# dguilliams3/book-recommendation-engine

Hardware: AMD Instinct MI355X
Metric: exact top-10 queries/sec at 10M×1536 fp32 (1/8 GPU) + % HBM/MFMA roofline (higher is better)
Workload: dtype fp32

## Files before the change

### book-recommendation-engine_amd/csrc/vs_api.hip

```cpp
#include <algorithm>
#include <cstdio>
#include <cstring>
#include <mutex>
#include <shared_mutex>
#include <string>
#include <vector>

#include "../../include/vsearch.h"
#include "vs_internal.h"

using namespace vs;

constexpr int kI8FirstBackoff = 8;
constexpr int kI8MaxBackoff = 64;

struct vs_index {
  int d = 0;
  int metric = VS_METRIC_L2;
  int dtype = VS_DTYPE_F32;
  int device = 0;
  int esize = 4;
  int64_t ld = 0;
  int64_t ntotal = 0;
  int64_t capacity = 0;
// ... 693 lines not shown
                           : (int)std::max<int64_t>(1, std::min<int64_t>(ntiles, (512 + nqt - 1) / nqt));
  part.P = 2 * nsplit;
  const size_t n = (size_t)a.nq_pad * part.P * KP;
  VS_HIP(scr.alloc((void**)&part.key, n * sizeof(float)), "vs: scratch");
  VS_HIP(scr.alloc((void**)&part.id, n * sizeof(int)), "vs: scratch");
  const void* qmat = a.qb16 ? a.qb16 : (const void*)a.qbuf;
  {
    KernelTimer tm(st, qlist ? nullptr : "gemm_topk");
    VS_HIP(launch_gemm_topk(KP, a.mode, idx->codes, a.xaux, qmat, a.qaux, idx->ld, idx->esize,
                            ntotal, a.nq_pad, nsplit, a.self0, part, st, qlist, qcount),
           "vs: gemm_topk launch");
    tm.stop();
  }
  VS_HIP(launch_merge_partials(a.mode, part, qlist ? a.nq_pad : a.nq, a.k, idx->id_base,
                               a.min_score, a.D, a.I, a.k, st, a.raw, qlist, qcount),
         "vs: merge launch");
  return VS_OK;
}

int adaptive_record(vs_index* idx, const int* handed, int n, hipStream_t st);
int run_paged(vs_index* idx, const SearchArgs& a, hipStream_t st, const int* gl = nullptr,
              const int* gc = nullptr);
int run_gemm_rescored(vs_index* idx, const SearchArgs& a, int need, int KF, int plane,
                      hipStream_t st, const int* gl, const int* gc);

static bool dump_enabled() {
  static const bool v = [] {
    const char* e = getenv("VS_X1_DUMP");
    return !e || atoi(e) != 0;
  }();
  return v;
}

static int recut_mode() {
  const char* e = getenv("VS_X1_RECUT");
  const int v = e ? atoi(e) : 1;
  return v == 0 ? 0 : v == 2 ? 2 : 1;
}

constexpr int64_t kSmallFilterMinRows = 1 << 18;
bool small_filter_on() {
  const char* e = getenv("VS_SMALL_FILTER");
  return !e || atoi(e) != 0;
}
bool small_l2d_ok(int mode, const SearchArgs& a) {
  if (!(mode == MODE_L2 && a.l2_direct)) return true;
  const char* e = getenv("VS_SMALL_L2D");
  return !e || atoi(e) != 0;
}

bool skinny_deep_on() {
  const char* e = getenv("VS_SKINNY_DEEP");
  return !e || atoi(e) != 0;
}

static int x1_wg_target(int nqt) {
  const char* e = getenv("VS_X1_WGS");
  const int v = e ? atoi(e) : 0;
  return v > 0 ? v : nqt <= 8 ? 256 : 512;
}

static bool tail_wait_on(const SearchArgs& a, hipStream_t st) {
  const char* e = getenv("VS_TAIL_WAIT");
  if (e && atoi(e) == 0) return false;
  if (a.host_wait) return true;
  hipStreamCaptureStatus cs = hipStreamCaptureStatusNone;
// ... 139 lines not shown
  }
  x.xaux = a.xaux;
  x.QH = QH;
  x.qs = qs;
  x.qaux = qaux;
  x.nqa = qa_rows;
  x.ld = !aug ? idx->ld : i8 ? idx->ld + idx->aug_m : idx->ld + kAugBf16;
  x.ntotal = ntotal;
  x.self0 = self_rows ? a.self0 : -1;
  x.qrow = qrow;
  x.qcount = gc;
  const BoundArgs ba = aug ? make_bound_args_l2aug(idx->ld, idx->aug, plane)
                           : make_bound_args(idx->ld, plane);
  if (!gathered && !small && x1_dump_applies(kmode, plane) && dump_enabled() &&
      x1_pass_dumps(ntotal, x.nsplit)) {
    const int64_t lists = (int64_t)x.nq_pad * part.P;
    const int dR = (int)std::min<int64_t>(x1_dump_slots(), (int64_t(4) << 30) / (lists * 8));
    if (dR >= 16) {
      int *dc = nullptr, *ds = nullptr;
      hipError_t e = scr.alloc((void**)&dc, (size_t)lists * sizeof(int));
      if (e == hipSuccess) e = scr.alloc((void**)&ds, (size_t)lists * dR * 2 * sizeof(int));
      if (e == hipSuccess) {
        VS_HIP(scr.alloc((void**)&x.qcut, (size_t)qa_rows * sizeof(float)), "vs: scratch");
        double* bk = nullptr;
        VS_HIP(scr.alloc((void**)&bk, (size_t)qa_rows * sizeof(double)), "vs: scratch");
        VS_HIP(hipMemsetD32Async((hipDeviceptr_t)x.qcut, 0x7f7fffff, (size_t)qa_rows, st),
               "vs: cuts");
        VS_HIP(hipMemsetAsync(dc, 0, (size_t)lists * sizeof(int), st), "vs: dumps");
        VS_HIP(launch_qbound(mode, Q, idx->ld, qaux, plane, stats, qr2, qa_rows, bk, st, &ba),
               "vs: cuts");
        x.qbkey = bk;
        x.qcut_m = need;
        x.dump = true;
        x.recut = recut_mode();
        x.dcount = dc;
        x.dslot = ds;
        x.dR = dR;
        x.dstats = device_stats(idx->device) ? device_stats(idx->device) + 6 : nullptr;
      } else {
        (void)hipGetLastError();
      }
    }
  }
  {
    KernelTimer whole(st, gathered ? nullptr : i8 ? "gemm_topk_x1_i8_pass" : "gemm_topk_x1_pass",
                      false);
    X1SpanTimer tm(i8 ? "gemm_topk_x1_i8" : "gemm_topk_x1",
                   i8 ? "gemm_topk_x1_i8_list" : "gemm_topk_x1_list");
    if (!gathered) x.timing = &tm;
    if (gathered && deep && !i8 && kmode == MODE_IP && a.self0 < 0 && skinny_deep_on()) {
      VS_HIP(launch_skinny_plane(FILTER_BF16, x.XH, x.QH, x.ld, ntotal, gc, nullptr, nullptr, part,
                                 st),
             "vs: skinny deep stage");
      x.qskip = skinny_plane_max_queries();
    }
    if (small) {
      int* cnt = nullptr;
      VS_HIP(scr.alloc((void**)&cnt, sizeof(int)), "vs: scratch");
      VS_HIP(hipMemsetD32Async((hipDeviceptr_t)cnt, a.nq, 1, st), "vs: count");
      KernelTimer ks(st, i8 ? "skinny_plane_topk_i8" : "skinny_plane_topk");
      VS_HIP(launch_skinny_plane(plane, x.XH, x.QH, x.ld, ntotal, cnt, qs, x.xs, part, st, a.nq),
             "vs: skinny first stage");
      ks.stop();
    } else {
      int nd = 0;
      VS_HIP(launch_gemm_topk_x1(kmode, x, part, st, &nd), "vs: gemm_topk_x1 launch");
// ... 1357 lines not shown
```

### book-recommendation-engine_amd/csrc/vs_gemm_x1.hip

```cpp
#include <algorithm>
#include <climits>
#include <cmath>
#include <cstdlib>
#include <type_traits>

#include "vs_device.h"

#ifndef VS_X1_PROBE
#define VS_X1_PROBE 0
#endif
#define VS_X1_P(bit) ((VS_X1_PROBE & (bit)) != 0)

namespace vs {

#ifndef VS_X1_STAMP
#define VS_X1_STAMP 0
#endif
constexpr int kStampSeg = 9;
constexpr int kStampCnt = 3;
constexpr int kStampN = 2 * (kStampSeg + kStampCnt) + 2;
__device__ unsigned long long g_x1_stamps[kStampN];

namespace {

constexpr int kT = 256;
constexpr int kNbuf = 5;
constexpr int kX1ChunkTiles = 64;
constexpr int kDumpMaxR = 128;
#ifndef VS_X1_SCHED_I8
#define VS_X1_SCHED_I8 0
#endif
#ifndef VS_X1_SEGDMA
#define VS_X1_SEGDMA 0
#endif
constexpr int x1_sched(int el, bool dump, bool hyb = false) {
  return el != FILTER_I8 ? 2 : VS_X1_SCHED_I8 ? VS_X1_SCHED_I8 : dump || hyb ? 2 : 1;
}
constexpr bool x1_has_dump(int mode, int el) {
  return mode == MODE_IP || (mode == MODE_COS && el == FILTER_I8);
}
static bool x1_cos_dump_on() {
  const char* e = getenv("VS_X1_COSDUMP");
  return e && atoi(e) != 0;
}

__device__ __forceinline__ unsigned long long stamp_now() {
  unsigned long long t;
  __builtin_amdgcn_sched_barrier(0);
  asm volatile("s_memtime %0\n\ts_waitcnt lgkmcnt(0)" : "=s"(t)::"memory");
  __builtin_amdgcn_sched_barrier(0);
  return t;
}

__device__ __forceinline__ f32x4 row4(const float* __restrict__ p) { return *(const f32x4*)p; }
__device__ __forceinline__ f32x4 row4(const uint16_t* __restrict__ p) {
  const uint2 u = *(const uint2*)p;
  return f32x4{__uint_as_float(u.x << 16), __uint_as_float(u.x & 0xFFFF0000u),
               __uint_as_float(u.y << 16), __uint_as_float(u.y & 0xFFFF0000u)};
}

__device__ __forceinline__ bf16x8 as_bf(const uint4& u) { return __builtin_bit_cast(bf16x8, u); }
__device__ __forceinline__ i32x4 as_i4(const uint4& u) { return __builtin_bit_cast(i32x4, u); }

template <int EL>
using AccT = typename std::conditional<EL == FILTER_I8, i32x16, f32x16>::type;
template <int EL>
__device__ __forceinline__ AccT<EL> mfma_blk(const uint4& a, const uint4& b, const AccT<EL>& c) {
  if constexpr (EL == FILTER_I8)
    return __builtin_amdgcn_mfma_i32_32x32x32_i8(as_i4(a), as_i4(b), c, 0, 0, 0);
  else
    return __builtin_amdgcn_mfma_f32_32x32x16_bf16(as_bf(a), as_bf(b), c, 0, 0, 0);
}

// ... 19 lines not shown
}

__device__ __forceinline__ float sel4x4(const f32x4 (&v)[4], int i) {
  float r = v[0][0];
#pragma unroll
  for (int j = 1; j < 16; ++j) r = i == j ? v[j >> 2][j & 3] : r;
  return r;
}

__device__ __forceinline__ int i8_threshold(float lim, float c) {
  const float q = lim * __builtin_amdgcn_rcpf(c);
  const float qm = q > 0.0f ? q * (1.0f - 0x1p-20f) : q * (1.0f + 0x1p-20f);
  float fl = floorf(qm) - 2.0f;
  fl = fminf(fmaxf(fl, -2147483520.0f), 2147483520.0f);
  const int T = (int)fl;
  return (float)T * c <= lim ? T : INT_MIN;
}

__device__ __forceinline__ float sel16(const f32x16& v, int i) {
  float r = v[0];
#pragma unroll
  for (int j = 1; j < 16; ++j) r = i == j ? v[j] : r;
  return r;
}

template <int EL>
__device__ __forceinline__ float x1_key(int sum_bits, float qsc, float fx) {
  if constexpr (EL == FILTER_I8) return -((float)sum_bits * (qsc * fx));
  else return -__int_as_float(sum_bits);
}

}

template <int KR, int MODE, bool DUMP, int EL, bool HYB = false>
__global__ __launch_bounds__(512, 1) void gemm_topk_x1(
    const char* __restrict__ XH, const float* __restrict__ xs, const float* __restrict__ xaux,
    const char* __restrict__ QH, const float* __restrict__ qs, const float* __restrict__ qaux,
    int nqa, int nksteps, int ntotal, int ntiles, int nsplit, int nqt, int qtile0, int64_t self0,
    const int* __restrict__ qrow, const int* __restrict__ qcount, int chunk, int chunk_end,
    int nchunk, int KP, int qg, float* __restrict__ pkey, int* __restrict__ pid,
    const float* __restrict__ xgmax, const float* __restrict__ xgmin, const float* __restrict__ qcut,
    int* __restrict__ dcount, int* __restrict__ dslot, int dR, int qskip) {
  static_assert(!DUMP || x1_has_dump(MODE, EL), "dump form");
  static_assert(!HYB || (!DUMP && x1_has_dump(MODE, EL)), "hybrid launch");
  constexpr int NBUF = kNbuf;
  constexpr int kStepB = kT * 64;
  constexpr int D = NBUF - 1;
  static_assert(NBUF * 2 * kStepB <= 160 * 1024, "LDS");
  __shared__ __attribute__((aligned(16))) char smem[NBUF * 2 * kStepB];

  const int tid = threadIdx.x;
  const int lane = tid & 63;
  const int w = __builtin_amdgcn_readfirstlane(tid >> 6);
  const int h = lane >> 5;
  const int c32 = lane & 31;
  const int wr = w & 1;
  const int wq = w >> 1;

  int qt, sp;
  {
    const int nblk = gridDim.x;
    const int b = blockIdx.x;
    const int qga = qg < 0 ? -qg : qg;
    const int QG = nqt < qga ? nqt : qga;
    const int G = nqt / QG;
    const int S = nblk >> 3;
    if ((nblk & 7) == 0 && nqt * nsplit == nblk && nqt % QG == 0 && G <= 8 && 8 % G == 0 &&
        S % QG == 0) {
      const int xcd = b & 7, slot = b >> 3, DG = S / QG;
      qt = (xcd % G) * QG + slot % QG;
      sp = (xcd / G) * DG + slot / QG;
    } else if (qg > 0 && (nblk & 7) == 0 && nqt * nsplit == nblk && nqt % QG == 0 && G % 8 == 0) {
      const int xcd = b & 7, slot = b >> 3, per = QG * nsplit;
      const int gi = slot / per, rem = slot - gi * per;
      qt = (gi * 8 + xcd) * QG + rem % QG;
      sp = rem / QG;
    } else {
      const int xcd = b & 7, slot = b >> 3, qq = nblk >> 3, rr = nblk & 7;
      const int lb = (xcd < rr ? xcd * (qq + 1) : rr * (qq + 1) + (xcd - rr) * qq) + slot;
      qt = lb % nqt;
      sp = lb / nqt;
    }
  }
  if (qcount && (qt * kT >= *qcount || *qcount <= qskip)) return;
  const int s0 = (int)((int64_t)sp * ntiles / nsplit);
  const int s1 = (int)((int64_t)(sp + 1) * ntiles / nsplit);
  const int t0 = s0 + (int)((int64_t)(s1 - s0) * chunk / nchunk);
  const int t1 = s0 + (int)((int64_t)(s1 - s0) * chunk_end / nchunk);
  const int tsw = HYB ? t0 + (t1 - t0 + 3) / 4 : t1;

  int gq[2], selfrow[2];
  float qa[2], qsc[2];
#pragma unroll
  for (int qb = 0; qb < 2; ++qb) {
    gq[qb] = qt * kT + 64 * wq + 32 * qb + c32;
    qa[qb] = 0.0f;
    if constexpr (MODE == MODE_L2 || (MODE == MODE_COS && EL != FILTER_I8))
      qa[qb] = gq[qb] < nqa ? qaux[gq[qb]] : 0.0f;
    qsc[qb] = 0.0f;
    if constexpr (EL == FILTER_I8) qsc[qb] = gq[qb] < nqa ? qs[gq[qb]] : 0.0f;
    selfrow[qb] = qrow ? (gq[qb] < nqa ? qrow[gq[qb]] : -1) : self0 >= 0 ? (int)(self0 + gq[qb]) : -1;
  }
  const int P = nsplit * 4;
  const int pl = sp * 4 + wr * 2 + h;
  constexpr int KL = KR;
  float lk[2][KL];
  int li[2][KL];
  float tq[2] = {0.0f, 0.0f};
  int dc[2] = {0, 0};
#pragma unroll
  for (int qb = 0; qb < 2; ++qb) {
    if constexpr (DUMP) {
      const int64_t o = ((int64_t)gq[qb] * P + pl) * KP + KR - 1;
      float tl = qcut[gq[qb]];
      if (pid[o] >= 0) tl = fminf(tl, pkey[o]);
      tq[qb] = gq[qb] < nqa ? tl : -FLT_MAX;
      dc[qb] = dcount[(int64_t)gq[qb] * P + pl];
      asm volatile("" ::"v"(tq[qb]), "v"(dc[qb]));
    } else {
      const int64_t o = ((int64_t)gq[qb] * P + pl) * KP;
      if (chunk == 0) {
        list_init<KR, int>(lk[qb], li[qb]);
      } else {
#pragma unroll
        for (int e = 0; e < KR; ++e) {
          lk[qb][e] = pkey[o + e];
          li[qb][e] = pid[o + e];
        }
      }
#pragma unroll
      for (int e = 0; e < KR; ++e) asm volatile("" ::"v"(lk[qb][e]), "v"(li[qb][e]));
    }
    asm volatile("" ::"v"(qa[qb]));
    if constexpr (EL == FILTER_I8) asm volatile("" ::"v"(qsc[qb]));
  }

  if (t1 > t0) {
    const uint32_t soff = (uint32_t)(lane >> 2) * 64u + (uint32_t)((lane & 3) ^ (lane >> 4)) * 16u;
    const int fsw = (c32 >> 2) & 3;
    const char* qtile = QH + (int64_t)(qtile0 + qt) * nksteps * kStepB + (uint32_t)(32 * w) * 64u;
    const uint32_t lds0 = (uint32_t)(uintptr_t)VS_LDS(smem);
    const int nsteps = (t1 - t0) * nksteps;

    int ls = 0, lt = t0, lk_ = 0, lbuf = 0;
    uint32_t xlane = 0;
    int xhi = 0;
    auto set_xoff = [&](int tt) {
      const int f = tile_perm(tt);
      const int ln = (int)__builtin_amdgcn_mbcnt_hi(~0u, __builtin_amdgcn_mbcnt_lo(~0u, 0u));
      xhi = f & 0xF0;
      xlane = (uint32_t)((ln >> 2) ^ (f & 0x0C)) * 64u + (uint32_t)((ln & 3) ^ (ln >> 4)) * 16u;
    };
    set_xoff(t0);
    constexpr bool kSeg = x1_sched(EL, DUMP, HYB) == 2 && MODE == MODE_IP;
    const char* xstep = nullptr;
    const char* qstep = nullptr;
    uint32_t xl0 = 0, xl2 = 0;
    auto set_step_ptrs = [&]() {
      const int r0 = (32 * w) ^ xhi, r2 = (32 * w + 16) ^ xhi;
      xstep = XH + ((int64_t)lt * nksteps + lk_) * kStepB + (uint32_t)(r0 & ~16) * 64u;
      qstep = qtile + (int64_t)lk_ * kStepB;
      xl0 = xlane + (uint32_t)(r0 & 16) * 64u;
      xl2 = xlane + (uint32_t)(r2 & 16) * 64u;
    };
    if constexpr (kSeg) set_step_ptrs();

    int Tq[2] = {0, 0};
    float fm = 0.0f, fn = FLT_MAX;
    auto set_Tq = [&]() {
#pragma unroll
      for (int qb = 0; qb < 2; ++qb) {
        const float c = qsc[qb] * fm, cn = qsc[qb] * fn, last = tq[qb];
        Tq[qb] = (c > 0.0f && -last >= 0.0f)                    ? i8_threshold(-last, c)
                 : (cn > 0.0f && cn <= FLT_MAX && -last < 0.0f) ? min(i8_threshold(-last, cn), -1)
                 : (c > 0.0f || -0.0f < last)                   ? INT_MIN
                                                                : INT_MAX;
        asm volatile("" ::"v"(Tq[qb]));
      }
    };
    auto set_factor_bounds = [&](int ta) {
      const int ln = (int)__builtin_amdgcn_mbcnt_hi(~0u, __builtin_amdgcn_mbcnt_lo(~0u, 0u));
      for (int g = 16 * ta + ln; g < 16 * t1; g += 64) {
        fm = fmaxf(fm, xgmax[g]);
        fn = fminf(fn, xgmin[g]);
      }
#pragma unroll
      for (int m = 32; m >= 1; m >>= 1) {
        fm = fmaxf(fm, __shfl_xor(fm, m));
        fn = fminf(fn, __shfl_xor(fn, m));
      }
    };
    if constexpr (DUMP && EL == FILTER_I8) {
      set_factor_bounds(t0);
      set_Tq();
    }
    auto to_dump_mode = [&]() {
      if constexpr (HYB) {
        const int ln = (int)__builtin_amdgcn_mbcnt_hi(~0u, __builtin_amdgcn_mbcnt_lo(~0u, 0u));
        const int pl1 = sp * 4 + wr * 2 + (ln >> 5);
#pragma unroll
        for (int qb = 0; qb < 2; ++qb) {
          const int64_t g = (int64_t)(qt * kT + 64 * wq + 32 * qb + (ln & 31)) * P + pl1;
          const int64_t o = g * KP;
#pragma unroll
// ... 16 lines not shown
        }
      }
    };

    AccT<EL> acc[4][2];
    uint4 fa0[4], fb0[2], fa1[4], fb1[2];
    auto rd = [&](int buf, int s2, uint4 (&fa)[4], uint4 (&fb)[2]) {
      const char* base = smem + buf * 2 * kStepB;
      const int co = ((2 * s2 + h) ^ fsw) * 16;
      const char* cX = base + (128 * wr + c32) * 64 + co;
      const char* cQ = base + kStepB + (64 * wq + c32) * 64 + co;
      if constexpr (!VS_X1_P(2)) {
        fb[0] = *(const uint4*)cQ;
        fb[1] = *(const uint4*)(cQ + 32 * 64);
#pragma unroll
        for (int rb = 0; rb < 4; ++rb) fa[rb] = *(const uint4*)(cX + rb * 32 * 64);
      } else {
        auto opq = [](uint4& u) { asm volatile("" : "+v"(u.x), "+v"(u.y), "+v"(u.z), "+v"(u.w)); };
        asm volatile("" ::"v"(cX), "v"(cQ));
        opq(fb[0]);
        opq(fb[1]);
#pragma unroll
        for (int rb = 0; rb < 4; ++rb) opq(fa[rb]);
      }
    };
    auto mfma_rb = [&](int rb, const uint4 (&fa)[4], const uint4 (&fb)[2]) {
      acc[rb][0] = mfma_blk<EL>(fa[rb], fb[0], acc[rb][0]);
      acc[rb][1] = mfma_blk<EL>(fa[rb], fb[1], acc[rb][1]);
    };
    auto mfma_rb_first = [&](int rb, const uint4 (&fa)[4], const uint4 (&fb)[2]) {
      const AccT<EL> z = {};
      acc[rb][0] = mfma_blk<EL>(fa[rb], fb[0], z);
      acc[rb][1] = mfma_blk<EL>(fa[rb], fb[1], z);
    };
    auto stage_piece = [&](int i) {
      const char* xbase = XH + ((int64_t)lt * nksteps + lk_) * kStepB +
                          (uint32_t)((32 * w + 16 * (i >> 1)) ^ xhi) * 64u;
      const char* qbase = qtile + (int64_t)lk_ * kStepB + (uint32_t)(16 * (i >> 1)) * 64u;
      const uint32_t lx = lds0 + (uint32_t)lbuf * (2 * kStepB) + (uint32_t)(2 * w) * 1024u;
      if constexpr (!VS_X1_P(1)) {
        if ((i & 1) == 0) {
          if constexpr (!VS_X1_P(16))
            glds16(xbase, xlane, __builtin_amdgcn_readfirstlane(lx + (i >> 1) * 1024u));
        } else {
          if constexpr (!VS_X1_P(32))
            glds16(qbase, soff, __builtin_amdgcn_readfirstlane(lx + kStepB + (i >> 1) * 1024u));
        }
      } else {
        asm volatile("" ::"v"(xlane), "v"(soff), "s"(xbase), "s"(qbase), "s"(lx));
      }
    };
    auto advance_cursor = [&]() {
      if (ls + 1 < nsteps) {
        ++ls;
        if constexpr (kSeg) {
          xstep += kStepB;
          qstep += kStepB;
        }
        if (++lk_ == nksteps) {
          lk_ = 0;
          set_xoff(++lt);
          if constexpr (kSeg) set_step_ptrs();
        }
      }
      lbuf = lbuf + 1 == NBUF ? 0 : lbuf + 1;
    };
// ... 216 lines not shown
                list_insert<KR, int>(lk[qb], li[qb], sel16(key, bi), row);
              }
            } else {
              const float last = lim(qb);
              if constexpr (EL == FILTER_I8) {
                const float c = qsc[qb] * fmx[rb];
                const int T = (c > 0.0f && -last >= 0.0f) ? i8_threshold(-last, c) : INT_MIN;
#pragma unroll
                for (int r = 0; r < 16; ++r) cm |= (uint32_t)(acc[rb][qb][r] > T) << r;
              } else {
#pragma unroll
                for (int r = 0; r < 16; ++r) cm |= (uint32_t)(-acc[rb][qb][r] < last) << r;
              }
              while (cm) {
                const int bi = __builtin_ctz(cm);
                cm &= cm - 1;
                const int row = rowof(rb, bi >> 2) + (bi & 3);
                float key;
                if constexpr (EL == FILTER_I8)
                  key = x1_key<EL>(sel16i(acc[rb][qb], bi), qsc[qb], sel4x4(rv[r2], bi));
                else
                  key = -sel16(acc[rb][qb], bi);
                const bool ok = (plain || (row < ntotal && row != selfrow[qb])) && key < lim(qb);
                if (ok) list_insert<KR, int>(lk[qb], li[qb], key, row);
              }
            }
          }
        }
        VS_X1_EMARK(8);
      }
      }
    };

    constexpr int kSched = x1_sched(EL, DUMP, HYB);
    if constexpr (kSched == 1) {

#pragma unroll
    for (int i = 0; i < D; ++i) {
#pragma unroll
      for (int j = 0; j < 4; ++j) stage_piece(j);
      advance_cursor();
    }
    asm volatile("s_waitcnt vmcnt(12)" ::: "memory");
    __builtin_amdgcn_s_barrier();
    asm volatile("" ::: "memory");
    rd(0, 0, fa0, fb0);
    int buf = 0;
    const bool lag = w >= 4;
#if VS_X1_STAMP
    tA = stamp_now();
#define VS_X1_MARK1(i) (tB = stamp_now(), sg[i] += tB - tA, tA = tB)
#else
#define VS_X1_MARK1(i) ((void)0)
#endif
    auto s1_step = [&](auto first_tag) {
      constexpr bool first = decltype(first_tag)::value;
      const int nbuf = buf + 1 == NBUF ? 0 : buf + 1;
      if (lag) {
        asm volatile("s_waitcnt vmcnt(8)" ::: "memory");
        __builtin_amdgcn_s_barrier();
      }
      __builtin_amdgcn_sched_barrier(0);
      if constexpr (first) {
        mfma_rb_first(0, fa0, fb0);
        __builtin_amdgcn_sched_barrier(0);
        rd(buf, 1, fa1, fb1);
// ... 46 lines not shown
        }
        VS_X1_MARK1(5);
      }
    };
    if constexpr (HYB) {
      s1_tiles(t0, tsw, std::false_type{});
      to_dump_mode();
      s1_tiles(tsw, t1, std::true_type{});
    } else {
      s1_tiles(t0, t1, std::integral_constant<bool, DUMP>{});
    }
#undef VS_X1_MARK1
    } else {
    static_assert(NBUF == 5, "segmented schedule: 3 steps in flight over 5 images");
#pragma unroll
    for (int i = 0; i < 3; ++i) {
      stage_step();
      advance_cursor();
    }
    asm volatile("s_waitcnt vmcnt(8)" ::: "memory");
    __builtin_amdgcn_s_barrier();
    const bool lag = w >= 4;
    if (lag) __builtin_amdgcn_s_barrier();
    int buf = 0;
#if VS_X1_STAMP
    tA = stamp_now();
#define VS_X1_MARK(i) (tB = stamp_now(), sg[i] += tB - tA, tA = tB)
#else
#define VS_X1_MARK(i) ((void)0)
#endif
    auto seg_step = [&](auto first_tag) {
      constexpr bool first = decltype(first_tag)::value;
      __builtin_amdgcn_sched_barrier(0);
      rd(buf, 0, fa0, fb0);
      rd(buf, 1, fa1, fb1);
      __builtin_amdgcn_sched_barrier(0);
#if !VS_X1_SEGDMA
      stage_step();
      advance_cursor();
      __builtin_amdgcn_sched_barrier(0);
      VS_X1_MARK(0);
      asm volatile("s_waitcnt vmcnt(8)" ::: "memory");
#else
      VS_X1_MARK(0);
      asm volatile("s_waitcnt vmcnt(4)" ::: "memory");
#endif
      VS_X1_MARK(1);
      __builtin_amdgcn_s_barrier();
      __builtin_amdgcn_sched_barrier(0);
      VS_X1_MARK(2);
#if !VS_X1_SEGDMA
      if constexpr (first) {
#pragma unroll
        for (int rb = 0; rb < 4; ++rb) mfma_rb_first(rb, fa0, fb0);
      } else {
#pragma unroll
        for (int rb = 0; rb < 4; ++rb) mfma_rb(rb, fa0, fb0);
      }
#pragma unroll
      for (int rb = 0; rb < 4; ++rb) mfma_rb(rb, fa1, fb1);
#else
      {
        const uint32_t lx = __builtin_amdgcn_readfirstlane(lds0 + (uint32_t)lbuf * (2 * kStepB) +
                                                           (uint32_t)(2 * w) * 1024u);
        auto piece = [&](int j, uint32_t m0v, uint32_t voff, const char* sbase) {
          if constexpr (!kSeg) {
            stage_piece(j);
            return;
          }
          uint32_t keep;
          asm volatile(
              "s_mov_b32 %0, m0\n\ts_mov_b32 m0, %1\n\ts_nop 0\n\t"
              "global_load_lds_dwordx4 %2, %3\n\ts_mov_b32 m0, %0"
              : "=&s"(keep)
              : "s"(m0v), "v"(voff), "s"(sbase)
              : "memory");
        };
        static_assert(kStepB == 0x4000, "piece offsets");
        if constexpr (first) {
          mfma_rb_first(0, fa0, fb0);
          mfma_rb_first(1, fa0, fb0);
        } else {
          mfma_rb(0, fa0, fb0);
          mfma_rb(1, fa0, fb0);
        }
        __builtin_amdgcn_sched_barrier(0);
        piece(0, lx, xl0, xstep);
        __builtin_amdgcn_sched_barrier(0);
        if constexpr (first) {
          mfma_rb_first(2, fa0, fb0);
          mfma_rb_first(3, fa0, fb0);
        } else {
          mfma_rb(2, fa0, fb0);
          mfma_rb(3, fa0, fb0);
        }
        __builtin_amdgcn_sched_barrier(0);
        piece(1, lx + 0x4000u, soff, qstep);
        __builtin_amdgcn_sched_barrier(0);
        mfma_rb(0, fa1, fb1);
        mfma_rb(1, fa1, fb1);
        __builtin_amdgcn_sched_barrier(0);
        piece(2, lx + 0x400u, xl2, xstep);
        __builtin_amdgcn_sched_barrier(0);
        mfma_rb(2, fa1, fb1);
        mfma_rb(3, fa1, fb1);
        __builtin_amdgcn_sched_barrier(0);
        piece(3, lx + 0x4400u, soff + 1024u, qstep);
        __builtin_amdgcn_sched_barrier(0);
        advance_cursor();
      }
#endif
      __builtin_amdgcn_sched_barrier(0);
      VS_X1_MARK(3);
      __builtin_amdgcn_s_barrier();
      __builtin_amdgcn_sched_barrier(0);
      VS_X1_MARK(4);
      VS_X1_MARK(5);
      buf = buf + 1 == NBUF ? 0 : buf + 1;
    };
    auto seg_tiles = [&](int ta, int tb, auto dm_tag) {
      for (int t = ta; t < tb; ++t) {
        seg_step(std::true_type{});
        for (int k = 1; k < nksteps; ++k) seg_step(std::false_type{});
        if constexpr (!VS_X1_P(8)) {
          epilogue(t, dm_tag);
        } else {
#pragma unroll
          for (int rb = 0; rb < 4; ++rb)
#pragma unroll
            for (int qb = 0; qb < 2; ++qb) asm volatile("" ::"v"(acc[rb][qb]));
        }
        VS_X1_MARK(5);
      }
    };
    if constexpr (HYB) {
      seg_tiles(t0, tsw, std::false_type{});
      to_dump_mode();
      seg_tiles(tsw, t1, std::true_type{});
    } else {
      seg_tiles(t0, t1, std::integral_constant<bool, DUMP>{});
    }
    if (!lag) __builtin_amdgcn_s_barrier();
#undef VS_X1_MARK
    }
#if VS_X1_STAMP
    {
      const int grp = w >= 4 ? 1 : 0;
      if (lane == 0) {
#pragma unroll
        for (int i = 0; i < kStampSeg; ++i)
          atomicAdd(&g_x1_stamps[grp * (kStampSeg + kStampCnt) + i], sg[i]);
        atomicAdd(&g_x1_stamps[2 * (kStampSeg + kStampCnt) + grp], (unsigned long long)nsteps);
      }
      if (lane == 0)
        atomicAdd(&g_x1_stamps[grp * (kStampSeg + kStampCnt) + kStampSeg], ecnt[0]);
    }
#endif
    asm volatile("s_waitcnt vmcnt(0)" ::: "memory");
  }

  const int ln = (int)__builtin_amdgcn_mbcnt_hi(~0u, __builtin_amdgcn_mbcnt_lo(~0u, 0u));
  const int pl0 = sp * 4 + wr * 2 + (ln >> 5);
#pragma unroll
  for (int qb = 0; qb < 2; ++qb) {
    const int64_t g = (int64_t)(qt * kT + 64 * wq + 32 * qb + (ln & 31)) * P + pl0;
    if (DUMP || (HYB && t1 > t0)) {
      dcount[g] = dc[qb];
    } else if (HYB) {
      const int64_t o = g * KP;
      for (int e = 0; e < KP; ++e) {
        pkey[o + e] = FLT_MAX;
        pid[o + e] = -1;
      }
    } else {
      const int64_t o = g * KP;
#pragma unroll
      for (int e = 0; e < KR; ++e) {
        pkey[o + e] = lk[qb][e];
        pid[o + e] = li[qb][e];
      }
      for (int e = KR; e < KP; ++e) {
        pkey[o + e] = FLT_MAX;
        pid[o + e] = -1;
      }
    }
  }
}

template <int KR, int EL>
__global__ __launch_bounds__(256) void x1_replay_kernel(
    int* __restrict__ dcount, const int* __restrict__ dslot, float* __restrict__ pkey,
    int* __restrict__ pid, int P, int KP, int nqa, const float* __restrict__ qs,
    const float* __restrict__ xs, int64_t self0, int ntotal, int dR, int64_t nl,
    float* __restrict__ qcut, unsigned long long* __restrict__ stats) {
  const int64_t i = (int64_t)blockIdx.x * 256 + threadIdx.x;
  const int cnt = i < (int64_t)nqa * P ? dcount[i] : 0;
  {
    unsigned long long a = (unsigned long long)cnt, b = cnt > dR ? 1ull : 0ull;
    for (int o = 32; o > 0; o >>= 1) {
// ... 106 lines not shown
  const int nqt = a.nq_pad / kT;
  const int per_block = (ntiles + a.nsplit - 1) / a.nsplit;
  const int qg = a.qcount ? nqt : x1_qg() * (x1_group_rounds() ? 1 : -1);
  const bool dump = a.dump && x1_has_dump(MODE, EL) && !a.qcount && a.qcut && a.qbkey &&
                    a.qcut_m > 0 && a.dcount && a.dslot && a.dR > 0;
  const int chunk_tiles = x1_chunk_tiles(per_block, dump);
  int nchunk = a.qcount ? 1 : std::max(1, (per_block + chunk_tiles - 1) / chunk_tiles);
  const int den = x1_split_den();
  const bool split = dump && nchunk < 4 && den >= 2 && per_block >= kSplitMinTiles;
  const bool cutting = dump && (nchunk >= 4 || split);
  const int tiles0 = (per_block + nchunk - 1) / nchunk;
  const bool hyb = dump && !split && x1_hybrid_on() && tiles0 >= kHybMinTiles;
  const bool later_dump = cutting || hyb;
  const int F = x1_first_den(EL);
  const bool quarter = cutting && !split && nchunk >= 4 && F >= 2 && per_block / (F * nchunk) >= 2;
  const bool sseg = split && x1_split_segments(den);
  int lg = 0;
  while ((1 << lg) < den) ++lg;
  const int nparts = split ? den : quarter ? F * nchunk : nchunk;
  const int nlaunch = sseg ? lg + 1 : split ? 2 : quarter ? nchunk + 1 : nchunk;
  const int64_t ldb = a.ld * filter_bytes(EL);
  if (a.qtile0 < 0) return hipErrorInvalidValue;
  for (int c = 0; c < nlaunch; ++c) {
    const int p0 = sseg    ? (c == 0 ? 0 : 1 << (c - 1))
                   : split   ? (c == 0 ? 0 : 1)
                   : quarter ? (c == 0 ? 0 : c == 1 ? 1 : F * (c - 1))
                             : c;
    const int p1 = sseg    ? (c == 0 ? 1 : 1 << c)
                   : split   ? (c == 0 ? 1 : den)
                   : quarter ? (c == 0 ? 1 : F * c)
                             : c + 1;
    if (a.timing)
      a.timing->begin(st, !(later_dump && nlaunch > 1) || c > 0, (double)(p1 - p0) / nparts);
    if (later_dump && c > 0) {
      if constexpr (x1_has_dump(MODE, EL))
        hipLaunchKernelGGL((gemm_topk_x1<KR, MODE, true, EL>), dim3(nqt * a.nsplit), dim3(512), 0,
                           st, (const char*)a.XH, a.xs, a.xaux, (const char*)a.QH, a.qs, a.qaux,
                           a.nqa, (int)(ldb / 64), a.ntotal, ntiles, a.nsplit, nqt, a.qtile0,
                           a.self0, a.qrow, a.qcount, p0, p1, nparts, part.KP, qg, part.key,
                           part.id, a.xgmax, a.xgmin, a.qcut, a.dcount, a.dslot, a.dR, a.qskip);
    } else if (hyb) {
      if constexpr (x1_has_dump(MODE, EL))
        hipLaunchKernelGGL((gemm_topk_x1<KR, MODE, false, EL, true>), dim3(nqt * a.nsplit),
                           dim3(512), 0, st, (const char*)a.XH, a.xs, a.xaux, (const char*)a.QH,
                           a.qs, a.qaux, a.nqa, (int)(ldb / 64), a.ntotal, ntiles, a.nsplit, nqt,
                           a.qtile0, a.self0, a.qrow, a.qcount, p0, p1, nparts, part.KP, qg,
                           part.key, part.id, a.xgmax, a.xgmin, a.qcut, a.dcount, a.dslot, a.dR, a.qskip);
    } else {
      hipLaunchKernelGGL((gemm_topk_x1<KR, MODE, false, EL>), dim3(nqt * a.nsplit), dim3(512), 0,
                         st, (const char*)a.XH, a.xs, a.xaux, (const char*)a.QH, a.qs, a.qaux,
                         a.nqa, (int)(ldb / 64), a.ntotal, ntiles, a.nsplit, nqt, a.qtile0,
                         a.self0, a.qrow, a.qcount, p0, p1, nparts, part.KP, qg, part.key,
                         part.id, a.xgmax, a.xgmin, nullptr, nullptr, nullptr, 0, a.qskip);
    }
    if (a.timing) a.timing->end(st);
    hipError_t e = hipGetLastError();
    if (e != hipSuccess) return e;
    if (hyb && c == 0) {
      e = launch_x1_replay(a, part, st);
      if (e != hipSuccess) return e;
    }
    if (cutting && c == 0) {
      e = launch_qcut(a, part, st);
      if (e != hipSuccess) return e;
    }
    if (later_dump && c > 0 && (sseg || ((c + 1) & c) == 0 || c + 1 == nlaunch)) {
      e = cutting && a.recut && c + 1 < nlaunch ? launch_x1_replay_cut(a, part, st)
// ... 1716 lines not shown
```

### book-recommendation-engine_amd/csrc/vs_internal.h

```cpp
#pragma once

#include <hip/hip_runtime.h>

#include <cfloat>
#include <climits>
#include <cstdint>

namespace vs {

enum Mode : int { MODE_IP = 0, MODE_L2 = 1, MODE_COS = 2, MODE_L2D = 3 };

constexpr int kBN = 128;
constexpr int kBQ = 128;
constexpr int kBK = 32;
constexpr int kRowPad = 256;
constexpr int kGemvMaxQ = 8;
constexpr int kBlasThreshold = 20;
constexpr int kSkinnyMaxQ = 32;

__host__ __device__ inline uint16_t f32_to_bf16_rne(float f) {
  uint32_t u;
  __builtin_memcpy(&u, &f, 4);
  if ((u & 0x7F800000u) == 0x7F800000u && (u & 0x007FFFFFu))
    return (uint16_t)((u >> 16) | 0x0040u);
// ... 15 lines not shown
                            const int* qlist = nullptr, const int* qcount = nullptr,
                            const float* fkey = nullptr, const int* fid = nullptr);
hipError_t launch_gemv_topk(int KP, int mode, int nq, const void* X, int esize, const float* Q,
                            int64_t ld, int ntotal, int nblocks, Partials part, hipStream_t st,
                            const float* fkey = nullptr, const int* fid = nullptr,
                            const int* run = nullptr);
hipError_t launch_skinny_plane(int filter, const void* XH, const void* QH, int64_t ld, int ntotal,
                               const int* qcount, const float* qs, const float* xs, Partials part,
                               hipStream_t st, int nq_hint = 0);
int skinny_plane_max_queries();
hipError_t launch_skinny_topk(int KP, int mode, int nq, const void* X, int esize,
                              const float* xaux, const void* Q, const float* qaux, int64_t ld,
                              int ntotal, int nblocks, Partials part, hipStream_t st,
                              const int* qcount = nullptr);
enum Filter : int { FILTER_BF16 = 0, FILTER_I8 = 1 };
inline int filter_bytes(int filter) { return filter == FILTER_I8 ? 1 : 2; }
__host__ __device__ inline int64_t plane_offset(int64_t row, int64_t byte, int64_t ldb) {
  return ((row >> 8) * (ldb >> 6) + (byte >> 6)) * 16384 + (row & 255) * 64 + (byte & 63);
}
struct X1Timing {
  virtual void begin(hipStream_t st, bool dominant, double share) = 0;
  virtual void end(hipStream_t st) = 0;
  virtual ~X1Timing() = default;
};
struct X1Args {
  X1Timing* timing = nullptr;
  int qskip = 0;
  int filter = FILTER_BF16;
  const void* XH = nullptr;
  const float* xs = nullptr;
  const float* xgmax = nullptr;
  const float* xgmin = nullptr;
  bool dump = false;
  float* qcut = nullptr;
  const double* qbkey = nullptr;
  int qcut_m = 0;
  int recut = 1;
  int* dcount = nullptr;
  int* dslot = nullptr;
  int dR = 0;
  unsigned long long* dstats = nullptr;
  const float* xaux = nullptr;
  const void* QH = nullptr;
  int qtile0 = 0;
  const float* qs = nullptr;
  const float* qaux = nullptr;
  int nqa = 0;
  int64_t ld = 0;
  int ntotal = 0;
  int nq_pad = 0;
  int nsplit = 1;
  int64_t self0 = -1;
  const int* qrow = nullptr;
  const int* qcount = nullptr;
};
constexpr int kX1Q = 256;
constexpr int64_t kI8MaxLd = 131072;
int x1_list_len(int need);
int x1_lane_len();
hipError_t x1_stamps(unsigned long long* out, int reset);
hipError_t launch_gemm_topk_x1(int mode, const X1Args& a, Partials part, hipStream_t st,
                               int* ndispatch);
struct BoundArgs {
  int filter = FILTER_BF16;
  double gam = 0.0;
  double norm_inf = 0.0;
// ... 146 lines not shown
```

Measured before the change: 82240.

## Use 16x16x64 i8 MFMA tiles for the dump-phase x1 kernel

Adds an S16 variant of the fused GEMM+top-k kernel for int8 inner-product dump launches. It reads LDS fragments in a 16-row layout, issues mfma_i32_16x16x64_i8 instead of the 32x32 form, and uses a matching epilogue that thresholds and dumps candidates. The aim is a cheaper MFMA shape and epilogue mapping for the later dump chunks. It is on by default unless VS_X1_DUMP_MFMA=32, and it changes the lane-to-query mapping and the dcount writes, which adds correctness risk.

```diff
diff --git a/book-recommendation-engine_amd/csrc/vs_api.hip b/book-recommendation-engine_amd/csrc/vs_api.hip
--- a/book-recommendation-engine_amd/csrc/vs_api.hip
+++ b/book-recommendation-engine_amd/csrc/vs_api.hip
@@ -749,6 +749,11 @@
   return v;
 }
 
+static bool dump_mfma32() {
+  const char* e = getenv("VS_X1_DUMP_MFMA");
+  return e && atoi(e) == 32;
+}
+
 static int recut_mode() {
   const char* e = getenv("VS_X1_RECUT");
   const int v = e ? atoi(e) : 1;
@@ -954,6 +959,7 @@
         x.qbkey = bk;
         x.qcut_m = need;
         x.dump = true;
+        x.dump32 = dump_mfma32();
         x.recut = recut_mode();
         x.dcount = dc;
         x.dslot = ds;
diff --git a/book-recommendation-engine_amd/csrc/vs_gemm_x1.hip b/book-recommendation-engine_amd/csrc/vs_gemm_x1.hip
--- a/book-recommendation-engine_amd/csrc/vs_gemm_x1.hip
+++ b/book-recommendation-engine_amd/csrc/vs_gemm_x1.hip
@@ -39,6 +39,9 @@
 constexpr bool x1_has_dump(int mode, int el) {
   return mode == MODE_IP || (mode == MODE_COS && el == FILTER_I8);
 }
+constexpr bool x1_has_s16(int mode, int el) {
+  return mode == MODE_IP && el == FILTER_I8 && x1_sched(el, true) == 2;
+}
 static bool x1_cos_dump_on() {
   const char* e = getenv("VS_X1_COSDUMP");
   return e && atoi(e) != 0;
@@ -124,7 +127,7 @@
 
 }
 
-template <int KR, int MODE, bool DUMP, int EL, bool HYB = false>
+template <int KR, int MODE, bool DUMP, int EL, bool HYB = false, bool S16 = false>
 __global__ __launch_bounds__(512, 1) void gemm_topk_x1(
     const char* __restrict__ XH, const float* __restrict__ xs, const float* __restrict__ xaux,
     const char* __restrict__ QH, const float* __restrict__ qs, const float* __restrict__ qaux,
@@ -135,6 +138,8 @@
     int* __restrict__ dcount, int* __restrict__ dslot, int dR, int qskip) {
   static_assert(!DUMP || x1_has_dump(MODE, EL), "dump form");
   static_assert(!HYB || (!DUMP && x1_has_dump(MODE, EL)), "hybrid launch");
+  static_assert(!S16 || (DUMP && !HYB && x1_has_s16(MODE, EL)), "16x16x64 form");
+  constexpr int NQB = S16 ? 4 : 2;
   constexpr int NBUF = kNbuf;
   constexpr int kStepB = kT * 64;
   constexpr int D = NBUF - 1;
@@ -181,11 +186,11 @@
   const int t1 = s0 + (int)((int64_t)(s1 - s0) * chunk_end / nchunk);
   const int tsw = HYB ? t0 + (t1 - t0 + 3) / 4 : t1;
 
-  int gq[2], selfrow[2];
-  float qa[2], qsc[2];
-#pragma unroll
-  for (int qb = 0; qb < 2; ++qb) {
-    gq[qb] = qt * kT + 64 * wq + 32 * qb + c32;
+  int gq[NQB], selfrow[NQB];
+  float qa[NQB], qsc[NQB];
+#pragma unroll
+  for (int qb = 0; qb < NQB; ++qb) {
+    gq[qb] = qt * kT + 64 * wq + (S16 ? 16 * qb + (lane & 15) : 32 * qb + c32);
     qa[qb] = 0.0f;
     if constexpr (MODE == MODE_L2 || (MODE == MODE_COS && EL != FILTER_I8))
       qa[qb] = gq[qb] < nqa ? qaux[gq[qb]] : 0.0f;
@@ -194,14 +199,14 @@
     selfrow[qb] = qrow ? (gq[qb] < nqa ? qrow[gq[qb]] : -1) : self0 >= 0 ? (int)(self0 + gq[qb]) : -1;
   }
   const int P = nsplit * 4;
-  const int pl = sp * 4 + wr * 2 + h;
+  const int pl = sp * 4 + wr * 2 + (S16 ? (lane >> 4) & 1 : h);
   constexpr int KL = KR;
   float lk[2][KL];
   int li[2][KL];
-  float tq[2] = {0.0f, 0.0f};
-  int dc[2] = {0, 0};
-#pragma unroll
-  for (int qb = 0; qb < 2; ++qb) {
+  float tq[NQB] = {};
+  int dc[NQB] = {};
+#pragma unroll
+  for (int qb = 0; qb < NQB; ++qb) {
     if constexpr (DUMP) {
       const int64_t o = ((int64_t)gq[qb] * P + pl) * KP + KR - 1;
       float tl = qcut[gq[qb]];
@@ -257,11 +262,11 @@
     };
     if constexpr (kSeg) set_step_ptrs();
 
-    int Tq[2] = {0, 0};
+    int Tq[NQB] = {};
     float fm = 0.0f, fn = FLT_MAX;
     auto set_Tq = [&]() {
 #pragma unroll
-      for (int qb = 0; qb < 2; ++qb) {
+      for (int qb = 0; qb < NQB; ++qb) {
         const float c = qsc[qb] * fm, cn = qsc[qb] * fn, last = tq[qb];
         Tq[qb] = (c > 0.0f && -last >= 0.0f)                    ? i8_threshold(-last, c)
                  : (cn > 0.0f && cn <= FLT_MAX && -last < 0.0f) ? min(i8_threshold(-last, cn), -1)
@@ -344,6 +349,42 @@
       const AccT<EL> z = {};
       acc[rb][0] = mfma_blk<EL>(fa[rb], fb[0], z);
       acc[rb][1] = mfma_blk<EL>(fa[rb], fb[1], z);
+    };
+    i32x4 acc16[S16 ? 8 : 1][4];
+    auto rd16 = [&](int buf) {
+      const char* base = smem + buf * 2 * kStepB;
+      const int c16 = lane & 15;
+      const int co = (((0x9C >> (2 * (lane >> 4))) & 3) ^ ((c16 >> 2) & 3)) * 16;
+      const char* cX = base + (128 * wr + c16) * 64 + co;
+      const char* cQ = base + kStepB + (64 * wq + c16) * 64 + co;
+      if constexpr (!VS_X1_P(2)) {
+        fb0[0] = *(const uint4*)cQ;
+        fb0[1] = *(const uint4*)(cQ + 16 * 64);
+        fb1[0] = *(const uint4*)(cQ + 32 * 64);
+        fb1[1] = *(const uint4*)(cQ + 48 * 64);
+#pragma unroll
+        for (int b = 0; b < 4; ++b) {
+          fa0[b] = *(const uint4*)(cX + b * 16 * 64);
+          fa1[b] = *(const uint4*)(cX + (b + 4) * 16 * 64);
+        }
+      } else {
+        auto opq = [](uint4& u) { asm volatile("" : "+v"(u.x), "+v"(u.y), "+v"(u.z), "+v"(u.w)); };
+        asm volatile("" ::"v"(cX), "v"(cQ));
+        opq(fb0[0]), opq(fb0[1]), opq(fb1[0]), opq(fb1[1]);
+#pragma unroll
+        for (int b = 0; b < 4; ++b) opq(fa0[b]), opq(fa1[b]);
+      }
+    };
+    auto mfma16_b = [&](int b, auto first_tag) {
+      if constexpr (S16) {
+        const uint4& a = b < 4 ? fa0[b & 3] : fa1[b & 3];
+#pragma unroll
+        for (int qb = 0; qb < 4; ++qb) {
+          const uint4& q = qb < 2 ? fb0[qb & 1] : fb1[qb & 1];
+          const i32x4 c = decltype(first_tag)::value ? i32x4{} : acc16[b][qb];
+          acc16[b][qb] = __builtin_amdgcn_mfma_i32_16x16x64_i8(as_i4(a), as_i4(q), c, 0, 0, 0);
+        }
+      }
     };
     auto stage_piece = [&](int i) {
       const char* xbase = XH + ((int64_t)lt * nksteps + lk_) * kStepB +
@@ -626,6 +667,64 @@
       }
     };
 
+    auto epilogue16 = [&](int t) {
+      if constexpr (S16) {
+        const bool plain = self0 < 0 && !qrow && (t + 1) * kT <= ntotal;
+        const int f = tile_perm(t);
+        const int fl = (4 * (lane >> 4)) ^ (f & 0x0C);
+        auto rowof16 = [&](int b) { return t * kT + ((128 * wr + 16 * b) ^ (f & 0xF0)) + fl; };
+        uint32_t pass = 0;
+#if VS_X1_STAMP
+        eA = stamp_now();
+#endif
+#pragma unroll
+        for (int qb = 0; qb < 4; ++qb) {
+          int amax = acc16[0][qb][0];
+#pragma unroll
+          for (int r = 1; r < 32; ++r) amax = max(amax, acc16[r >> 2][qb][r & 3]);
+          pass |= (uint32_t)(amax > Tq[qb]) << qb;
+        }
+        VS_X1_EMARK(6);
+        if constexpr (VS_X1_P(128)) {
+          asm volatile("" ::"v"(pass));
+          pass = 0;
+        }
+        if (__ballot(pass != 0) != 0) {
+          const int64_t nl = (int64_t)nqt * kT * P;
+#pragma unroll
+          for (int qb = 0; qb < 4; ++qb) {
+            if (__ballot((pass >> qb) & 1u) == 0) continue;
+            int* const dst = dslot + ((int64_t)gq[qb] * P + pl) * 2;
+#pragma unroll
+            for (int b = 0; b < 8; ++b) {
+              uint32_t cm = 0;
+#pragma unroll
+              for (int e = 0; e < 4; ++e) cm |= (uint32_t)(acc16[b][qb][e] > Tq[qb]) << e;
+              const int row0 = rowof16(b);
+              if (!plain) {
+#pragma unroll
+                for (int e = 0; e < 4; ++e)
+                  if (!(row0 + e < ntotal && row0 + e != selfrow[qb])) cm &= ~(1u << e);
+              }
+              if (__ballot(cm != 0) == 0) continue;
+              const int n = __popc(cm);
+              const int np = __shfl_xor(n, 32);
+              int c = dc[qb] + (lane >= 32 ? np : 0);
+              dc[qb] += n + np;
+#pragma unroll
+              for (int e = 0; e < 4; ++e) {
+                if (cm & (1u << e)) {
+                  if (c < dR) *(i32x2*)(dst + (int64_t)c * nl * 2) = i32x2{row0 + e, acc16[b][qb][e]};
+                  ++c;
+                }
+              }
+            }
+          }
+        }
+        VS_X1_EMARK(8);
+      }
+    };
+
     constexpr int kSched = x1_sched(EL, DUMP, HYB);
     if constexpr (kSched == 1) {
 
@@ -738,8 +837,12 @@
     auto seg_step = [&](auto first_tag) {
       constexpr bool first = decltype(first_tag)::value;
       __builtin_amdgcn_sched_barrier(0);
-      rd(buf, 0, fa0, fb0);
-      rd(buf, 1, fa1, fb1);
+      if constexpr (S16) {
+        rd16(buf);
+      } else {
+        rd(buf, 0, fa0, fb0);
+        rd(buf, 1, fa1, fb1);
+      }
       __builtin_amdgcn_sched_barrier(0);
 #if !VS_X1_SEGDMA
       stage_step();
@@ -756,15 +859,20 @@
       __builtin_amdgcn_sched_barrier(0);
       VS_X1_MARK(2);
 #if !VS_X1_SEGDMA
-      if constexpr (first) {
-#pragma unroll
-        for (int rb = 0; rb < 4; ++rb) mfma_rb_first(rb, fa0, fb0);
+      if constexpr (S16) {
+#pragma unroll
+        for (int b = 0; b < 8; ++b) mfma16_b(b, first_tag);
       } else {
-#pragma unroll
-        for (int rb = 0; rb < 4; ++rb) mfma_rb(rb, fa0, fb0);
-      }
-#pragma unroll
-      for (int rb = 0; rb < 4; ++rb) mfma_rb(rb, fa1, fb1);
+        if constexpr (first) {
+#pragma unroll
+          for (int rb = 0; rb < 4; ++rb) mfma_rb_first(rb, fa0, fb0);
+        } else {
+#pragma unroll
+          for (int rb = 0; rb < 4; ++rb) mfma_rb(rb, fa0, fb0);
+        }
+#pragma unroll
+        for (int rb = 0; rb < 4; ++rb) mfma_rb(rb, fa1, fb1);
+      }
 #else
       {
         const uint32_t lx = __builtin_amdgcn_readfirstlane(lds0 + (uint32_t)lbuf * (2 * kStepB) +
@@ -783,7 +891,10 @@
               : "memory");
         };
         static_assert(kStepB == 0x4000, "piece offsets");
-        if constexpr (first) {
+        if constexpr (S16) {
+          mfma16_b(0, first_tag);
+          mfma16_b(1, first_tag);
+        } else if constexpr (first) {
           mfma_rb_first(0, fa0, fb0);
           mfma_rb_first(1, fa0, fb0);
         } else {
@@ -793,7 +904,10 @@
         __builtin_amdgcn_sched_barrier(0);
         piece(0, lx, xl0, xstep);
         __builtin_amdgcn_sched_barrier(0);
-        if constexpr (first) {
+        if constexpr (S16) {
+          mfma16_b(2, first_tag);
+          mfma16_b(3, first_tag);
+        } else if constexpr (first) {
           mfma_rb_first(2, fa0, fb0);
           mfma_rb_first(3, fa0, fb0);
         } else {
@@ -803,13 +917,23 @@
         __builtin_amdgcn_sched_barrier(0);
         piece(1, lx + 0x4000u, soff, qstep);
         __builtin_amdgcn_sched_barrier(0);
-        mfma_rb(0, fa1, fb1);
-        mfma_rb(1, fa1, fb1);
+        if constexpr (S16) {
+          mfma16_b(4, first_tag);
+          mfma16_b(5, first_tag);
+        } else {
+          mfma_rb(0, fa1, fb1);
+          mfma_rb(1, fa1, fb1);
+        }
         __builtin_amdgcn_sched_barrier(0);
         piece(2, lx + 0x400u, xl2, xstep);
         __builtin_amdgcn_sched_barrier(0);
-        mfma_rb(2, fa1, fb1);
-        mfma_rb(3, fa1, fb1);
+        if constexpr (S16) {
+          mfma16_b(6, first_tag);
+          mfma16_b(7, first_tag);
+        } else {
+          mfma_rb(2, fa1, fb1);
+          mfma_rb(3, fa1, fb1);
+        }
         __builtin_amdgcn_sched_barrier(0);
         piece(3, lx + 0x4400u, soff + 1024u, qstep);
         __builtin_amdgcn_sched_barrier(0);
@@ -829,7 +953,13 @@
         seg_step(std::true_type{});
         for (int k = 1; k < nksteps; ++k) seg_step(std::false_type{});
         if constexpr (!VS_X1_P(8)) {
-          epilogue(t, dm_tag);
+          if constexpr (S16) epilogue16(t);
+          else epilogue(t, dm_tag);
+        } else if constexpr (S16) {
+#pragma unroll
+          for (int b = 0; b < 8; ++b)
+#pragma unroll
+            for (int qb = 0; qb < 4; ++qb) asm volatile("" ::"v"(acc16[b][qb]));
         } else {
 #pragma unroll
           for (int rb = 0; rb < 4; ++rb)
@@ -866,11 +996,14 @@
   }
 
   const int ln = (int)__builtin_amdgcn_mbcnt_hi(~0u, __builtin_amdgcn_mbcnt_lo(~0u, 0u));
-  const int pl0 = sp * 4 + wr * 2 + (ln >> 5);
-#pragma unroll
-  for (int qb = 0; qb < 2; ++qb) {
-    const int64_t g = (int64_t)(qt * kT + 64 * wq + 32 * qb + (ln & 31)) * P + pl0;
-    if (DUMP || (HYB && t1 > t0)) {
+  const int pl0 = sp * 4 + wr * 2 + (S16 ? (ln >> 4) & 1 : ln >> 5);
+#pragma unroll
+  for (int qb = 0; qb < NQB; ++qb) {
+    const int64_t g =
+        (int64_t)(qt * kT + 64 * wq + (S16 ? 16 * qb + (ln & 15) : 32 * qb + (ln & 31))) * P + pl0;
+    if constexpr (S16) {
+      if (ln < 32) dcount[g] = dc[qb];
+    } else if (DUMP || (HYB && t1 > t0)) {
       dcount[g] = dc[qb];
     } else if (HYB) {
       const int64_t o = g * KP;
@@ -1043,7 +1176,15 @@
                              : c + 1;
     if (a.timing)
       a.timing->begin(st, !(later_dump && nlaunch > 1) || c > 0, (double)(p1 - p0) / nparts);
-    if (later_dump && c > 0) {
+    if (later_dump && c > 0 && x1_has_s16(MODE, EL) && !a.dump32) {
+      if constexpr (x1_has_s16(MODE, EL))
+        hipLaunchKernelGGL((gemm_topk_x1<KR, MODE, true, EL, false, true>), dim3(nqt * a.nsplit),
+                           dim3(512), 0, st, (const char*)a.XH, a.xs, a.xaux, (const char*)a.QH,
+                           a.qs, a.qaux, a.nqa, (int)(ldb / 64), a.ntotal, ntiles, a.nsplit, nqt,
+                           a.qtile0, a.self0, a.qrow, a.qcount, p0, p1, nparts, part.KP, qg,
+                           part.key, part.id, a.xgmax, a.xgmin, a.qcut, a.dcount, a.dslot, a.dR,
+                           a.qskip);
+    } else if (later_dump && c > 0) {
       if constexpr (x1_has_dump(MODE, EL))
         hipLaunchKernelGGL((gemm_topk_x1<KR, MODE, true, EL>), dim3(nqt * a.nsplit), dim3(512), 0,
                            st, (const char*)a.XH, a.xs, a.xaux, (const char*)a.QH, a.qs, a.qaux,
diff --git a/book-recommendation-engine_amd/csrc/vs_internal.h b/book-recommendation-engine_amd/csrc/vs_internal.h
--- a/book-recommendation-engine_amd/csrc/vs_internal.h
+++ b/book-recommendation-engine_amd/csrc/vs_internal.h
@@ -71,6 +71,7 @@
   const float* xgmax = nullptr;
   const float* xgmin = nullptr;
   bool dump = false;
+  bool dump32 = false;
   float* qcut = nullptr;
   const double* qbkey = nullptr;
   int qcut_m = 0;
```

Result: faster. 84880 (median of 6 runs) (+3.2%).
